# mariohsouto/ProxSDP.jl

Hardware: AMD Instinct MI355X
Metric: PDHG iterations/sec at target rank ~ sqrt(n), Max-Cut SDP n=4000 (tol 1e-4 options) (higher is better)
Workload: dtype f64

## Files before the change

### include/proxsdp_hip.h

```cpp
#ifndef PROXSDP_HIP_H
#define PROXSDP_HIP_H

#include <stdint.h>

#ifdef __cplusplus
extern "C" {
#endif

#define PROXSDP_HIP_ABI_VERSION 10

#define PROXSDP_E_INVALID  (-1)
#define PROXSDP_E_HIP      (-2)
#define PROXSDP_E_NOMEM    (-3)
#define PROXSDP_E_UNSUPP   (-4)
#define PROXSDP_E_INTERNAL (-5)
#define PROXSDP_E_COMM_ABORTED (-6)

#define PROXSDP_STATUS_NOT_CALLED       0
#define PROXSDP_STATUS_OPTIMAL          1
#define PROXSDP_STATUS_TIME_LIMIT       2
#define PROXSDP_STATUS_ITERATION_LIMIT  3
#define PROXSDP_STATUS_INFEAS_OR_UNBND  4
#define PROXSDP_STATUS_DUAL_INFEASIBLE  5
#define PROXSDP_STATUS_INFEASIBLE       6
// ... 265 lines not shown
                            double* packed_out, int32_t* out_rank, double* out_min_eig,
                            int64_t* out_nmatvec, int32_t* out_converged, int32_t* out_fell_back);

int proxsdp_hip_eigsolve(const double* packed, int64_t n, int32_t nev,
                         const proxsdp_options* opt, const double* resid, int32_t cap,
                         double* vals, double* vecs, int32_t* out_count,
                         int32_t* out_converged, int64_t* out_nmatvec, int32_t* out_numiter);

int proxsdp_hip_symv_packed(const double* packed, int64_t n, const double* v, double* y,
                            int32_t repeat, double* ms);

int proxsdp_hip_reconstruct(const double* Z, const double* lambda, int64_t n, int32_t r,
                            double* packed_out, int32_t repeat, double* ms);
int proxsdp_hip_reconstruct_kernel(const double* Z, const double* lambda, int64_t n, int32_t r, int32_t mfma,
                                   double* packed_out, int32_t repeat, double* ms);

int proxsdp_hip_factor_residual(const double* packed, int64_t n, const double* V, int64_t ldv,
                                const double* lam, int32_t r, double* resid2, double* xnorm2);
int proxsdp_hip_factor_residual_kernel(const double* packed, int64_t n, const double* V, int64_t ldv,
                                       const double* lam, int32_t r, double* resid2, double* xnorm2,
                                       int32_t repeat, double* ms);

int proxsdp_hip_full_eig_kernel(const double* packed_in, int64_t n, int32_t sign, double* packed_out,
                                int32_t repeat, double* ms, int32_t* out_rank, int64_t* out_products);

int proxsdp_hip_spmv(const proxsdp_csc* M, int32_t index_base, int32_t transpose,
                     const double* in, double* out);

int proxsdp_hip_primal_update(const double* x, const double* Mty, const double* c, double tau, int64_t n,
                              double* x_out);
// ... 95 lines not shown
```

### proxsdp.jl_amd/binding.py

```python
import ctypes as C
import os
import pathlib
import re

import numpy as np
import scipy.sparse as sp

_HERE = pathlib.Path(__file__).resolve().parent
LIB_PATH = _HERE / "libproxsdp_hip.so"
HEADER_PATH = _HERE.parent / "include" / "proxsdp_hip.h"

TRACE_COLS = 14
TRACE_NAMES = ("iter", "prim_obj", "dual_obj", "gap", "feas", "prim_res", "dual_res",
               "primal_step", "beta", "theta", "target_rank", "trials", "elapsed", "matvecs")


class LibraryNotBuilt(RuntimeError):
    pass


class ProxSDPHipError(RuntimeError):
    def __init__(self, code, msg):
        super().__init__(f"libproxsdp_hip error {code}: {msg}")
        self.code = code
# ... 704 lines not shown
                                   int(p), len(b[0]), float(sigma), _p(out)))
    return out


def reconstruct(Z, lam, n, repeat=0, mfma=-1):
    L = lib()
    Zc = np.asfortranarray(Z, dtype=np.float64)
    lam = _f(lam)
    r = len(lam)
    out = np.zeros(n * (n + 1) // 2)
    ms = f64(0.0)
    _check(L.proxsdp_hip_reconstruct_kernel(Zc.ctypes.data_as(pf64), _p(lam), n, r, mfma, _p(out), repeat, C.byref(ms)))
    return (out, ms.value) if repeat else out


def factor_residual(packed, n, V, lam, repeat=0):
    L = lib()
    x = _f(packed)
    lam = _f(lam)
    r = len(lam)
    Vc = np.asfortranarray(np.asarray(V, dtype=np.float64).reshape(-1, r) if r else np.zeros((n, 0)))
    ldv = Vc.shape[0] if r else n
    if len(x) != n * (n + 1) // 2 or (r and ldv < n):
        raise ValueError("factor_residual: packed / V have the wrong shape")
    r2, x2, ms = f64(0.0), f64(0.0), f64(0.0)
    _check(L.proxsdp_hip_factor_residual_kernel(_p(x), n, Vc.ctypes.data_as(pf64) if r else None, ldv,
                                                _p(lam) if r else None, r, C.byref(r2), C.byref(x2), int(repeat), C.byref(ms)))
    return (r2.value, x2.value, ms.value) if repeat else (r2.value, x2.value)


# ... 238 lines not shown
```

### proxsdp.jl_amd/csrc/capi.hip

```cpp
#include <functional>
#include <memory>
#include <new>
#include <string>

#include "pdhg_loop.hip.hpp"
#include "shard_split.hpp"

namespace {
thread_local std::string g_last_error;

template <typename F>
int guarded(F&& f) {
    try {
        g_last_error.clear();
        return f();
    } catch (const std::bad_alloc&) {
        g_last_error = "out of memory";
        return PROXSDP_E_NOMEM;
    } catch (const proxsdp::HipError& e) {
        g_last_error = e.what();
        return PROXSDP_E_HIP;
    } catch (const std::invalid_argument& e) {
        g_last_error = e.what();
        return PROXSDP_E_INVALID;
// ... 601 lines not shown
            hipEvent_t a, b;
            PX_HIP(hipEventCreate(&a)); PX_HIP(hipEventCreate(&b));
            PX_HIP(hipEventRecord(a, S.stream));
            for (int i = 0; i < repeat; ++i) S.launch_reconstruct(W, Zd.p, (int)n, ld.p, r, x.p);
            PX_HIP(hipEventRecord(b, S.stream));
            PX_HIP(hipEventSynchronize(b));
            float t = 0.f;
            PX_HIP(hipEventElapsedTime(&t, a, b));
            *ms = (double)t / repeat;
            (void)hipEventDestroy(a); (void)hipEventDestroy(b);
        }
        return 0;
    });
}

int proxsdp_hip_factor_residual(const double* packed, int64_t n, const double* V, int64_t ldv,
                                const double* lam, int32_t r, double* resid2, double* xnorm2) {
    return proxsdp_hip_factor_residual_kernel(packed, n, V, ldv, lam, r, resid2, xnorm2, 0, nullptr);
}

int proxsdp_hip_factor_residual_kernel(const double* packed, int64_t n, const double* V, int64_t ldv,
                                       const double* lam, int32_t r, double* resid2, double* xnorm2,
                                       int32_t repeat, double* ms) {
    return guarded([&]() -> int {
        if (!packed || !resid2 || !xnorm2 || (r > 0 && (!V || !lam))) throw std::invalid_argument("NULL buffer");
        if (r < 0) throw std::invalid_argument("r < 0");
        if (n < 1 || n > 46340) throw std::invalid_argument("n out of range");
        if (r > 0 && (ldv < n || ldv >= (int64_t)1 << 31)) throw std::invalid_argument("ldv out of range");
        Engine E(nullptr, n, 2);
        proxsdp::Solver& S = E.S;
// ... 366 lines not shown
```

### proxsdp.jl_amd/csrc/kernels.hip.hpp

```cpp
#pragma once
#include <hip/hip_runtime.h>
#include <cstdint>

namespace proxsdp {
namespace dev {

constexpr int WAVE = 64;
constexpr int TILE = 64;
constexpr int TPB = 256;
constexpr int NWAVE = TPB / WAVE;
constexpr int CPW = TILE / NWAVE;
constexpr double INV_SQRT2 = 0.70710678118654752440;
constexpr double SQRT2 = 1.41421356237309504880;

#ifdef PX_TIMELINE
constexpr int TL_WG = 160, TL_SLOTS = 8, TL_K = 260;
__device__ unsigned long long g_tl[2][TL_K][TL_WG][TL_SLOTS];
#define PX_TL(kind, k, slot)                                                                                   \
    do {                                                                                                       \
        if (threadIdx.x == 0 && (int)blockIdx.x < ::proxsdp::dev::TL_WG && (k) >= 0 && (k) < ::proxsdp::dev::TL_K) { \
            asm volatile("" ::: "memory");                                                                     \
            ::proxsdp::dev::g_tl[kind][k][blockIdx.x][slot] = wall_clock64();                                    \
            asm volatile("" ::: "memory");                                                                     \
        }                                                                                                      \
// ... 1013 lines not shown
                }
            }
        }
    }
    if (FUSE_RES) {
        const double r0 = block_max(m0, s_red);
        const double r1 = block_max(m1, s_red);
        if (threadIdx.x == 0) { respart[blockIdx.x] = r0; respart[rstride + blockIdx.x] = r1; }
    }
}

typedef double v4f64 __attribute__((ext_vector_type(4)));
constexpr int MF_KC = 16;
constexpr int MF_LD = TILE + 16;
template <bool FUSE_RES>
__global__ void __launch_bounds__(TPB)
k_reconstruct_mfma(const double* __restrict__ Z, int ldz, const double* __restrict__ lam, int r,
                   int n, double* __restrict__ xp, const double* __restrict__ xold,
                   const unsigned* __restrict__ mask, long long mask_off, double* __restrict__ respart,
                   int rstride) {
    __shared__ double sA[2][MF_KC][MF_LD];
    __shared__ double sB[2][MF_KC][MF_LD];
    __shared__ double s_red[NWAVE];
    const int nt_ = (n + TILE - 1) / TILE;
    const int tile = xcd_tile(blockIdx.x, nt_ * (nt_ + 1) / 2);
    if (tile >= nt_ * (nt_ + 1) / 2) return;
    int I, J;
    tile_coords(tile, I, J);
    const int lane = threadIdx.x & 63;
    const int w = __builtin_amdgcn_readfirstlane((int)(threadIdx.x >> 6));
    const int l15 = lane & 15, l4 = lane >> 4;
    const int gja = J * TILE + lane, gib = I * TILE + lane;
    const bool ja_ok = gja < n, ib_ok = gib < n;
    const double* __restrict__ zA = Z + (ja_ok ? gja : 0);
    const double* __restrict__ zB = Z + (ib_ok ? gib : 0);
    constexpr int MF_U = MF_KC / NWAVE;
    double pa[MF_U], pb[MF_U];
    auto fetch = [&](int k0) {
#pragma unroll
        for (int u = 0; u < MF_U; ++u) {
            const int k = k0 + w + 4 * u;
            const bool kok = k < r;
            const long long ko = (long long)(kok ? k : 0) * ldz;
            const double lk = lam[kok ? k : 0];
            pa[u] = (kok && ja_ok) ? zA[ko] * lk : 0.0;
            pb[u] = (kok && ib_ok) ? zB[ko] : 0.0;
        }
    };
    auto stash = [&](int buf) {
#pragma unroll
        for (int u = 0; u < MF_U; ++u) { sA[buf][w + 4 * u][lane] = pa[u]; sB[buf][w + 4 * u][lane] = pb[u]; }
    };
    v4f64 acc[4];
#pragma unroll
    for (int b = 0; b < 4; ++b) acc[b] = (v4f64){0.0, 0.0, 0.0, 0.0};
    double xo[16];
    unsigned mk[16];
    if (FUSE_RES) {
#pragma unroll
        for (int reg = 0; reg < 4; ++reg) {
            const int gjc = min(J * TILE + w * 16 + l4 + 4 * reg, n - 1);
#pragma unroll
            for (int b = 0; b < 4; ++b) {
                const int gic = min(I * TILE + b * 16 + l15, gjc);
                const long long idxc = (long long)gjc * (gjc + 1) / 2 + gic;
                xo[reg * 4 + b] = xold[idxc];
                mk[reg * 4 + b] = mask[(mask_off + idxc) >> 5];
            }
        }
    }
    fetch(0);
    stash(0);
    __syncthreads();
    int cur = 0;
    for (int k0 = 0; k0 < r; k0 += MF_KC) {
        const bool more = k0 + MF_KC < r;
        if (more) fetch(k0 + MF_KC);
#pragma unroll
        for (int q = 0; q < MF_KC / 4; ++q) {
            const double a = sA[cur][4 * q + l4][w * 16 + l15];
            double bv[4];
#pragma unroll
            for (int b = 0; b < 4; ++b) bv[b] = sB[cur][4 * q + l4][b * 16 + l15];
#pragma unroll
            for (int b = 0; b < 4; ++b) acc[b] = __builtin_amdgcn_mfma_f64_16x16x4f64(a, bv[b], acc[b], 0, 0, 0);
        }
        if (more) {
            stash(cur ^ 1);
            __syncthreads();
            cur ^= 1;
        }
    }
    double m0 = 0.0, m1 = 0.0;
#pragma unroll
    for (int reg = 0; reg < 4; ++reg) {
        const int gj = J * TILE + w * 16 + l4 + 4 * reg;
#pragma unroll
        for (int b = 0; b < 4; ++b) {
            const int gi = I * TILE + b * 16 + l15;
            if (gj < n && gi <= gj) {
                const long long idx = (long long)gj * (gj + 1) / 2 + gi;
                const double xn = ((gi == gj) ? 1.0 : SQRT2) * acc[b][reg];
                if (FUSE_RES) {
                    const double xov = xo[reg * 4 + b];
                    const long long gidx = mask_off + idx;
                    const bool on = (mk[reg * 4 + b] >> (gidx & 31)) & 1u;
                    if (!on) { m0 = fmax(m0, fabs(xn - xov)); m1 = fmax(m1, fabs(xov)); }
                }
                xp[idx] = xn;
            }
        }
    }
    if (FUSE_RES) {
        const double r0 = block_max(m0, s_red);
        const double r1 = block_max(m1, s_red);
        if (threadIdx.x == 0) { respart[blockIdx.x] = r0; respart[rstride + blockIdx.x] = r1; }
    }
}

__global__ void __launch_bounds__(TPB)
k_factor_residual(const double* __restrict__ xp, int n, const double* __restrict__ V, int ldv,
                  const double* __restrict__ lam, int r, double* __restrict__ part) {
    __shared__ double sA[2][MF_KC][MF_LD];
    __shared__ double sB[2][MF_KC][MF_LD];
    __shared__ double s_red[NWAVE];
    const int nt_ = (n + TILE - 1) / TILE;
    const int tile = xcd_tile(blockIdx.x, nt_ * (nt_ + 1) / 2);
    if (tile >= nt_ * (nt_ + 1) / 2) return;
    int I, J;
    tile_coords(tile, I, J);
// ... 68 lines not shown
                const double d = x - acc[b][reg];
                s0 += wt * (d * d);
                s1 += wt * (x * x);
            }
        }
    }
    const double r0 = block_sum(s0, s_red);
    const double r1 = block_sum(s1, s_red);
    if (threadIdx.x == 0) { part[2 * tile] = r0; part[2 * tile + 1] = r1; }
}

constexpr int RM_LDV = TILE + 16;
constexpr int RM_CG = 16;
__global__ void __launch_bounds__(TPB)
k_lz_rotate_mfma(const double* __restrict__ V, int ldv, int K, const double* __restrict__ U, int ncols,
                 double* __restrict__ out, int ldo, int copy_src, int copy_dst) {
    extern __shared__ double s_mem[];
    const int Kp = (K + 3) & ~3;
    const int ldu = Kp + 2;
    double* s_V = s_mem;
    double* s_U = s_mem + (size_t)Kp * RM_LDV;
    const int lane = threadIdx.x & 63;
    const int w = __builtin_amdgcn_readfirstlane((int)(threadIdx.x >> 6));
    const int l15 = lane & 15, l4 = lane >> 4;
    const int i0 = blockIdx.x * LZ_ROWS;
    const int c0 = blockIdx.y * RM_CG;
    const int cn = min(RM_CG, ncols - c0);
    if (cn > 0) {
        double tu[RM_CG / NWAVE][2];
        for (int jb = 0; jb < Kp; jb += 2 * WAVE) {
#pragma unroll
// ... 26 lines not shown
        }
        __syncthreads();
        v4f64 acc = (v4f64){0.0, 0.0, 0.0, 0.0};
        for (int q = 0; q < Kp / 4; ++q) {
            const double bv = s_V[(4 * q + l4) * RM_LDV + w * 16 + l15];
            const double av = s_U[l15 * ldu + 4 * q + l4];
            acc = __builtin_amdgcn_mfma_f64_16x16x4f64(av, bv, acc, 0, 0, 0);
        }
#pragma unroll
        for (int reg = 0; reg < 4; ++reg) {
            const int c = l4 + 4 * reg;
            if (c < cn) out[(long long)(c0 + c) * ldo + i0 + w * 16 + l15] = acc[reg];
        }
    }
    if (copy_src >= 0 && blockIdx.y == 0 && w == 0) out[(long long)copy_dst * ldo + i0 + lane] = V[(long long)copy_src * ldv + i0 + lane];
}

__global__ void __launch_bounds__(TPB)
k_small_psd_project(double* __restrict__ x, const long long* __restrict__ offs, const int* __restrict__ sides,
                    double tol_psd, int* __restrict__ rank_out, int* __restrict__ npos_out, int nmin, int nmax) {
    extern __shared__ __attribute__((aligned(16))) double sj_mem[];
    __shared__ double s_red[NWAVE];
    __shared__ int s_cnt[2];
    const int n = sides[blockIdx.x];
    if (n < nmin || n > nmax) return;
    double* __restrict__ xp = x + offs[blockIdx.x];
    const int ld = n | 1;
    double* A = sj_mem;
    double* V = A + n * ld;
    double* cs = V + n * ld;
// ... 845 lines not shown
```

### proxsdp.jl_amd/csrc/pdhg_loop.hip.hpp

```cpp
#pragma once
#include "solver.hip.hpp"

namespace proxsdp {

constexpr int PSTRIDE = 2048;
constexpr int NQ = 16;

inline void Solver::spmv(const double* x, double* y) {
    spmv_sparse(x, y);
    if (P.dense()) dense_mv(x, y, true);
}
inline void Solver::spmv_sparse(const double* x, double* y) {
    if (P.Q == 0) return;
    if (csr_wave)
        hipLaunchKernelGGL(dev::k_spmv_csr_wave, dim3(ceil_div(P.Q, dev::NWAVE)), dim3(dev::TPB), 0, stream,
                           csr_ptr.p, csr_col.p, csr_val.p, x, y, (int)P.Q, LONG_ROW);
    else
        hipLaunchKernelGGL(dev::k_spmv_csr_thread, dim3(ceil_div(P.Q, dev::TPB)), dim3(dev::TPB), 0, stream,
                           csr_ptr.p, csr_col.p, csr_val.p, x, y, (int)P.Q, LONG_ROW);
    if (n_seg > 0) {
        hipLaunchKernelGGL(dev::k_spmv_csr_seg, dim3(n_seg), dim3(dev::TPB), 0, stream,
                           seg_lo_d.p, seg_hi_d.p, csr_col.p, csr_val.p, x, segpart_d.p);
        hipLaunchKernelGGL(dev::k_spmv_seg_fin, dim3(ceil_div(n_long, dev::TPB)), dim3(dev::TPB), 0, stream,
                           long_row_d.p, long_ptr_d.p, n_long, segpart_d.p, y);
// ... 142 lines not shown
        return;
    }
    double mn = W.vals[0];
    for (double v : W.vals) mn = std::min(mn, v);
    min_eig[idx] = mn;
    int first = 0, npos = 0;
    if (opt.eigsolver == 1) {
        for (int i = 0; i < nev; ++i) if (W.vals[i] > 0.0) ++npos;
        first = nev - npos;
    } else {
        const int k = std::min(nev, W.converged_eigs);
        for (int i = 0; i < k; ++i) if (W.vals[i] > 0.0) ++npos;
    }
    current_rank[idx] += npos;
    W.last_npos = npos;
    if (npos > 0) W.lam.upload(W.vals.data() + first, npos, stream);
    launch_reconstruct(W, W.Z.p + (size_t)first * W.npad, W.npad, W.lam.p, npos, xo,
                       fuse ? xp : nullptr, fuse ? idx : -1);
    W.recon_r += npos;
    if (W.fop_ok) {
        std::swap(W.Z.p, W.F.p);
        W.F_first = first; W.F_r = npos;
        std::swap(W.lam.p, W.Flam.p);
        std::swap(W.lam.n, W.Flam.n);
        W.have_factors = true; W.x_prev_sparse = false;
    } else {
        W.ritz_first = first; W.ritz_r = npos; W.ritz_ok = true;
    }
    if (W.sign_check_pending) verify_sign_engine(idx, xo);
}

// ... 129 lines not shown
                    if (debug) std::fprintf(stderr, "[proxsdp] certificate failed: block %d iteration %lld theta %.3e scale %.3e npos %d\n",
                                            idx, (long long)iter, theta, cscale, npos);
                    break;
                }
                W.lst.full_eigs_lanczos_certified++;
            }
        }
        int rank = 0;
        for (int i = 0; i < npos; ++i) if (W.vals[i] > opt.tol_psd) ++rank;
        W.use_fop = false;
        if (used_fop) W.lst.fop_projections++;
        W.lst.full_eigs++; W.lst.full_eigs_lanczos++;
        current_rank[idx] = rank;
        min_eig[idx] = 0.0;
        W.last_npos = npos;
        if (npos > 0) W.lam.upload(W.vals.data(), npos, stream);
        launch_reconstruct(W, W.Z.p, W.npad, W.lam.p, npos, xo, fuse ? xp : nullptr, fuse ? idx : -1);
        W.recon_r += npos;
        if (W.fop_ok) {
            std::swap(W.Z.p, W.F.p);
            W.F_first = 0; W.F_r = npos;
            std::swap(W.lam.p, W.Flam.p);
            std::swap(W.lam.n, W.Flam.n);
            W.have_factors = true; W.x_prev_sparse = false;
        } else {
            W.ritz_first = 0; W.ritz_r = npos; W.ritz_ok = true;
        }
        if (verify) {
            if (W.sg_cmp.n < 2) W.sg_cmp.alloc(2);
            W.sg_cmp.zero(stream);
            hipLaunchKernelGGL(dev::k_maxdiff, dim3(grid_for(W.N)), dim3(dev::TPB), 0, stream, (const double*)xo,
// ... 1572 lines not shown
```

### proxsdp.jl_amd/csrc/solver.hip.hpp

```cpp
#pragma once
#include <hip/hip_runtime.h>
#include <hip/hip_ext.h>
#include <array>
#include <memory>
#include <mutex>
#include <condition_variable>
#include <functional>
#include <exception>
#include <rocblas/rocblas.h>
#include <rocsolver/rocsolver.h>

#include <algorithm>
#include <chrono>
#include <cmath>
#include <cstdio>
#include <cstdlib>
#include <cstring>
#include <stdexcept>
#include <string>
#include <thread>
#include <tuple>
#include <type_traits>
#include <utility>
#include <vector>
// ... 108 lines not shown
    }
};

struct EigEvents {
    std::vector<hipEvent_t> e0, e1;
    size_t used = 0;
    std::pair<hipEvent_t, hipEvent_t> acquire() {
        if (used == e0.size()) {
            hipEvent_t a, b;
            PX_HIP(hipEventCreate(&a)); PX_HIP(hipEventCreate(&b));
            e0.push_back(a); e1.push_back(b);
        }
        ++used;
        return {e0[used - 1], e1[used - 1]};
    }
    void harvest(double& ms_sum, int64_t& count) {
        for (size_t s = 0; s < used; ++s) {
            float ms = 0.f;
            if (hipEventElapsedTime(&ms, e0[s], e1[s]) == hipSuccess) { ms_sum += ms; count++; }
        }
        used = 0;
    }
};

struct StreamRef {
    hipStream_t main = nullptr;
    static inline thread_local hipStream_t tl = nullptr;
    operator hipStream_t() const { return tl ? tl : main; }
};

struct LzRun {
    int nev = 0, krylovdim = 0, ld = 0;
    bool arpack = false, positive_part = false;
    double tol = 0.0, step_tol = 0.0;
    long long maxiter = 0;
    std::vector<double> T, Tw, D, U, f, al, be, Qa, da, ea;
// ... 37 lines not shown
    PinnedBuf Ustage[2];
    int ustage_next = 0;
    std::vector<double> vals;
    int count = 0, converged_eigs = 0, numiter = 0, prev_numiter = 1;
    bool converged = false;
    DevBuf<double> F, Flam, tpart, ebuf, apartf;
    DevBuf<int> ell_col, ell_sidx;
    DevBuf<int> wr_ptr, wr_row, wr_lo, wr_hi, ov_col, ov_sidx;
    dev::EllOverflow ov{};
    int ell_w = 0, F_first = 0, F_r = 0;
    bool fop_ok = false;
    bool have_factors = false;
    bool x_prev_sparse = true;
    bool use_fop = false;
    bool ritz_ok = false;
    int ritz_first = 0, ritz_r = 0;
    int last_npos = -1;
    hipStream_t side = nullptr;
    hipEvent_t ev_mid = nullptr, ev_early = nullptr;
    PinnedBuf rec_early;
    SplitEig split;
    int batch_slot = 0;
    bool b1_defer = false;
    int b1_rot_K = 0;
    const double* b1_rot_U = nullptr;
    LzRun lzrun;
    long long fel_served = 0;
    bool fel_disabled = false;
    int fel_cert_fails = 0;
    DevBuf<double> warm_part;
// ... 136 lines not shown
    int block1_lds_cap = 0;
    DevBuf<long long> b1_dbg;
    bool block1_plan(const EigWork& W, int krylovdim, bool split_wanted) const;
    void launch_block1(EigWork& W, const double* xp, int kfirst, int krylovdim, double tol);
    bool sg48_ok = false;
    void launch_symv(EigWork& W, const double* xp, const double* v, bool use_ctl, dev::LanczosCtl* ctl = nullptr);
    void launch_symv_finish(EigWork& W, const double* xp, int kclose, double tol, bool use_carry);
    void launch_reconstruct(EigWork& W, const double* Z, int ldz, const double* lam, int r, double* xp_out,
                            const double* xp_old = nullptr, int blk = -1);
    proxsdp_psd_factors* factors_out = nullptr;
    DevBuf<double> fac_V, fac_lam, fac_part;
    void factor_residual(const double* xp, int n, const double* V, int ldv, const double* lam, int r,
                         double& resid2, double& xnorm2);
    void extract_factors(const std::vector<double>& x);
    void rotate(EigWork& W, int K, const std::vector<double>& U, int ldu, int ncols, double* out, int copy_src, int copy_dst,
                const double* extra, int nextra);

    void test_project(int idx, double* xp, int tr);
    void test_full_eig(const double* xin, double* xout) { current_rank.assign(1, 0); min_eig.assign(1, 0.0); full_eig_project(0, xin, xout, false); }
    long long test_rank() const { return current_rank.empty() ? 0 : current_rank[0]; }
    double test_min_eig() const { return min_eig.empty() ? 0.0 : min_eig[0]; }
    void test_spmv(bool transpose, const double* in, double* out);
    void test_trial_batch(proxsdp_trial_batch& t);
    void test_cone_tail(const double* x, int64_t n, const int64_t* so, const int32_t* sl, int nsoc,
                        const int64_t* oo, int none, double* x_soc, double* gap_in, double* gap_out,
                        double* x_clamp, double* mineig);
    void test_sym_product(proxsdp_sym_product& t);
    void test_sign_unpack(const double* packed, double sentinel, double* A, double* sc);

    bool debug = std::getenv("PROXSDP_HIP_DEBUG") != nullptr;
    proxsdp_options opt;
// ... 475 lines not shown
                                    double& resid2, double& xnorm2) {
    const int nt = ceil_div(n, dev::TILE);
    const int tiles = nt * (nt + 1) / 2;
    if (fac_part.n < (size_t)2 * tiles) fac_part.alloc((size_t)2 * tiles);
    hipLaunchKernelGGL(dev::k_factor_residual, dim3(8 * ceil_div(tiles, 8)), dim3(dev::TPB), 0, stream,
                       xp, n, V, ldv, lam, r, fac_part.p);
    PX_HIP(hipGetLastError());
    std::vector<double> h((size_t)2 * tiles);
    fac_part.download(h.data(), h.size(), stream);
    PX_HIP(hipStreamSynchronize(stream));
    resid2 = 0.0; xnorm2 = 0.0;
    for (int t = 0; t < tiles; ++t) { resid2 += h[2 * t]; xnorm2 += h[2 * t + 1]; }
}

inline void Solver::rotate(EigWork& W, int K, const std::vector<double>& U, int ldu, int ncols,
                           double* out, int copy_src, int copy_dst, const double* extra, int nextra) {
    if (rot_sink != nullptr) {
        RotSink::Req& q = rot_sink->slot[W.batch_slot];
        q.W = &W; q.V = W.V.p; q.out = out; q.K = K; q.ncols = ncols; q.copy_src = copy_src; q.copy_dst = copy_dst;
        q.nextra = std::max(nextra, 0); q.valid = true;
        q.data.resize((size_t)K * std::max(ncols, 0) + (size_t)q.nextra);
        for (int c = 0; c < ncols; ++c)
            for (int j = 0; j < K; ++j) q.data[(size_t)c * K + j] = U[(size_t)c * ldu + j];
        for (int t = 0; t < q.nextra; ++t) q.data[(size_t)K * std::max(ncols, 0) + t] = extra[t];
        return;
    }
    double* tmp = W.Ustage[W.ustage_next].p;
    W.ustage_next ^= 1;
    if ((size_t)K * std::max(ncols, 1) + (size_t)std::max(nextra, 0) > W.ustage_doubles)
        throw std::logic_error("rotation staging buffer too small");
    for (int c = 0; c < ncols; ++c)
        for (int j = 0; j < K; ++j) tmp[(size_t)c * K + j] = U[(size_t)c * ldu + j];
    for (int q = 0; q < nextra; ++q) tmp[(size_t)K * ncols + q] = extra[q];
    if (W.b1_defer && nextra > 0 && K < 32 && copy_src == K && copy_dst == ncols && out == W.Z.p) {
        W.b1_rot_K = K; W.b1_rot_U = tmp;
        W.arrow_p = tmp + (size_t)K * ncols;
        return;
    }
    W.U.upload(tmp, (size_t)K * ncols + (size_t)std::max(nextra, 0), stream);
    if (nextra > 0) W.arrow_p = W.U.p + (size_t)K * ncols;
    if (W.lzrun.wide) {
        if (ncols > 0 || copy_src >= 0)
            hipLaunchKernelGGL(dev::k_lzw_rotate, dim3(W.nt, std::max(1, ceil_div(ncols, dev::LZW_RC))), dim3(dev::TPB), 0, stream,
                               (const double*)W.V.p, W.npad, K, (const double*)W.U.p, ncols, out, W.npad, copy_src, copy_dst);
        return;
    }
    {
        const int Kp = (K + 3) & ~3;
        const size_t lds_m = ((size_t)Kp * dev::RM_LDV + (size_t)dev::RM_CG * (Kp + 2)) * sizeof(double);
        if (K >= 32 && ncols >= 16 && (int)lds_m <= rotate_mfma_lds_cap) {
            hipLaunchKernelGGL(dev::k_lz_rotate_mfma, dim3(W.nt, ceil_div(ncols, dev::RM_CG)), dim3(dev::TPB), lds_m, stream,
                               (const double*)W.V.p, W.npad, K, (const double*)W.U.p, ncols, out, W.npad, copy_src, copy_dst);
            return;
        }
    }
    const int vbytes = K * (dev::LZ_ROWS + 1) * 8;
    const int maxcols = std::max(1, (rotate_lds_cap - vbytes) / (8 * K));
    int c0 = 0;
    do {
        const int cn = std::max(0, std::min(maxcols, ncols - c0));
        const bool last = (c0 + cn >= ncols);
        if (cn > 0 || (last && copy_src >= 0))
            hipLaunchKernelGGL(dev::k_lz_rotate, dim3(W.nt), dim3(dev::TPB), (size_t)K * cn * 8 + vbytes, stream,
                               W.V.p, W.npad, W.n, K, W.U.p + (size_t)c0 * K, K, cn,
                               out + (size_t)c0 * W.npad, W.npad, last ? copy_src : -1, copy_dst - c0);
        c0 += std::max(cn, 1);
    } while (c0 < ncols);
}

// ... 165 lines not shown
    }
    R.kfirst = keep;
    R.presymv = speculated;
    ++R.numiter;
    W.lst.lanczos_restarts++;
}

inline void Solver::lz_finish_run(EigWork& W, LzRun& R) {
    const int K = R.K, nev = R.nev;
    W.numiter = R.numiter;
    if (R.positive_part) {
        if (R.pos_fail || R.pos_count < 0) { W.converged = false; return; }
        W.count = R.pos_count; W.converged_eigs = R.pos_count; W.converged = true;
        W.vals.assign(R.D.begin(), R.D.begin() + R.pos_count);
        if (R.pos_count > 0 && R.merge_active) lz_merge_vectors(W, R, R.pos_count);
        if (R.pos_count > 0) rotate(W, K, R.U, K, R.pos_count, W.Z.p, -1, 0, nullptr, 0);
        return;
    }
    if (R.pos_fail) { W.converged = false; return; }
    if (R.arpack) {
        W.converged_eigs = R.converged;
        if (R.converged < nev) { W.converged = false; return; }
        W.count = nev;
        W.vals.assign(R.D.begin(), R.D.begin() + nev);
        std::reverse(W.vals.begin(), W.vals.end());
        std::vector<double> Ur((size_t)K * nev);
        for (int c = 0; c < nev; ++c)
            for (int r = 0; r < K; ++r) Ur[(size_t)c * K + r] = R.U[(size_t)(nev - 1 - c) * K + r];
        rotate(W, K, Ur, K, nev, W.Z.p, -1, 0, nullptr, 0);
        W.converged = true;
        return;
    }
    int howmany = R.howmany;
    if (R.converged > howmany) howmany = R.converged;
    W.count = howmany;
    W.vals.assign(R.D.begin(), R.D.begin() + howmany);
    W.converged_eigs = R.converged;
    W.converged = (R.converged != 0);
    if (R.merge_active) lz_merge_vectors(W, R, howmany);
    rotate(W, K, R.U, K, howmany, W.Z.p, -1, 0, nullptr, 0);
}

inline void Solver::lanczos_eager(EigWork& W, const double* xp, int nev) {
    LzRun& R = W.lzrun;
    W.use_fop = false;
    if (!lz_init(W, R, nev, false)) return;
    if (R.arpack) throw std::invalid_argument("krylovkit_eager applies to eigsolver = 2 (KrylovKit) only");
    if (R.wide) throw std::invalid_argument("krylovkit_eager: Krylov dimension > 255 is not supported");
    const int kd = R.krylovdim, ld = R.ld;
    const double tol = R.tol;
    lz_launch_begin(W, W.resid.p, W.ctl_p);
    std::vector<double>& T = R.T; std::vector<double>& f = R.f;
    std::vector<double> fstep(2 * dev::MAXK, 0.0);
    int K = 0, kfirst = 0, converged = 0;
    double beta = 0.0;
// ... 144 lines not shown
    std::vector<double> T((size_t)msteps * msteps, 0.0), d(msteps, 0.0);
    for (int j = 0; j < msteps; ++j) {
        if (!(al[j] == al[j]) || !(j + 1 < msteps ? be[j] == be[j] : true)) return false;
        T[(size_t)j * msteps + j] = al[j];
        if (j + 1 < msteps) T[(size_t)j * msteps + j + 1] = T[(size_t)(j + 1) * msteps + j] = be[j];
    }
    if (msteps == 1) d[0] = al[0];
    else if (symeig_dense(msteps, T.data(), d.data(), true) != 0) return false;
    theta_max = d[msteps - 1];
    scale = std::max({std::fabs(d[0]), std::fabs(theta_max), npos > 0 ? std::fabs(W.vals[0]) : 0.0});
    return true;
}

inline void Solver::lanczos(EigWork& W, const double* xp, int nev, bool positive_part) {
    W.ritz_ok = false;
    if (opt.krylovkit_eager && opt.eigsolver != 1 && !positive_part) { lanczos_eager(W, xp, nev); return; }
    LzRun& R = W.lzrun;
    if (!lz_init(W, R, nev, positive_part)) return;
    const int krylovdim = R.krylovdim;
    const double step_tol = R.step_tol;
    const bool wide = R.wide;
    if (wide) W.lst.wide_krylov_projections++;
    if (krylovdim >= 96) QlPool::get().arm();
    dev::LanczosCtl* const ctl = wide ? W.ctlw_p : W.ctl_p;
    const bool warm_start = positive_part ? (opt.lanczos_warm_start >= 0) : (opt.lanczos_warm_start > 0);
    if (!wide && warm_start && W.fop_ok && W.have_factors && W.F_r > 0 && W.tpart.n > 0) {
        const int nb = ceil_div(W.npad, dev::TPB);
        hipLaunchKernelGGL(dev::k_lz_warm_sum, dim3(nb), dim3(dev::TPB), 0, stream,
                           W.V.p, (const double*)(W.F.p + (size_t)W.F_first * W.npad), W.npad, W.F_r,
                           (const double*)W.resid.p, W.npad, W.warm_part.p,
// ... 19 lines not shown
        pool_guard.p = merge_pool.get();
        W.split.M.par = &merge_par;
        W.split.M.nchunk = merge_helpers() + 1;
    }
    if (use_split && W.side == nullptr) {
        PX_HIP(hipStreamCreateWithFlags(&W.side, hipStreamNonBlocking));
        PX_HIP(hipEventCreateWithFlags(&W.ev_mid, hipEventDisableTiming));
        PX_HIP(hipEventCreateWithFlags(&W.ev_early, hipEventDisableTiming));
        W.rec_early.alloc(EigWork::REC_DOUBLES);
    }
    struct DeferGuard {
        EigWork& W;
        DeferGuard(EigWork& w, bool on) : W(w) { W.b1_defer = on; }
        ~DeferGuard() { W.b1_defer = false; }
    };
    while (true) {
        const int kfirst = R.kfirst;
        const int k1 = (kfirst == 0) ? (18 * krylovdim) / 25 : kfirst + 1;
        const bool split_cycle = use_split && k1 >= 1 && k1 <= krylovdim - 2;
        if (wide) {
            for (int k = kfirst; k < krylovdim; ++k) lzw_step(W, xp, k, kfirst, step_tol, R.presymv);
        } else if (blk1) {
            launch_block1(W, xp, kfirst, krylovdim, step_tol);
            R.presymv = false;
        } else {
            for (int k = kfirst; k < krylovdim; ++k) {
                lz_launch_step(W, xp, k, kfirst, step_tol, R.presymv);
                if (split_cycle && k == k1) {
                    PX_HIP(hipEventRecord(W.ev_mid, stream));
                    PX_HIP(hipStreamWaitEvent(W.side, W.ev_mid, 0));
// ... 2 lines not shown
                }
            }
            lz_launch_finish(W, krylovdim - 1, step_tol, krylovdim - 1 > kfirst);
        }
        const bool speculate = !blk1 && (W.prev_numiter > 1 || R.numiter > 1);
        if (speculate) {
            launch_symv(W, xp, W.V.p + (size_t)krylovdim * W.npad, true, ctl);
            count_matvecs(W, -1);
        }
        if (wide) PX_HIP(hipMemcpyAsync(W.recw_pinned.p, W.recw.p, EigWork::RECW_DOUBLES * sizeof(double), hipMemcpyDeviceToHost, stream));
        else PX_HIP(hipMemcpyAsync(W.rec_host, W.rec.p, EigWork::REC_DOUBLES * sizeof(double), hipMemcpyDeviceToHost, stream));
        if (!(split_cycle && lz_split_first(W, R, k1))) lz_prepare_arrow(R);
        const double tdbg0 = debug ? now_s() : 0.0;
        wait_stream();
        if (debug) { dbg_lz[0] += now_s() - tdbg0; dbg_lz[5] += 1.0; }
        if (W.cye_pending) {
            W.cye_pending = false;
            float ms = 0.f;
            if (hipEventElapsedTime(&ms, W.cye[0], W.cye[1]) == hipSuccess) W.lst.cycle_ms += ms;
        }
        W.ev.harvest(W.lst.symv_profiled_ms, W.lst.symv_profiled);
        W.evo.harvest(W.lst.orth_profiled_ms, W.lst.orth_profiled);
        const double tdbg1 = debug ? now_s() : 0.0;
        bool go_on;
        {
            DeferGuard defer(W, blk1);
            go_on = lz_after_cycle(W, R, speculate);
        }
        if (debug) dbg_lz[1] += now_s() - tdbg1;
        if (!go_on) break;
    }
    const double tdbg2 = debug ? now_s() : 0.0;
    lz_finish_run(W, R);
    if (debug) dbg_lz[3] += now_s() - tdbg2;
}

inline void Solver::lzw_step(EigWork& W, const double* xp, int k, int kfirst, double step_tol, bool& presymv) {
    if (k == kfirst && presymv) {
        count_matvecs(W, 1);
    } else {
        launch_symv(W, xp, W.V.p + (size_t)k * W.npad, true, W.ctlw_p);
    }
    presymv = false;
    const dev::LanczosCtl* ctl = W.ctlw_p;
    const int nred = ceil_div(k + 2, dev::TPB);
    hipLaunchKernelGGL(dev::k_lzw_dots, dim3(W.nt), dim3(dev::TPB), 0, stream,
                       (const double*)W.Ppart.p, W.nt, W.npad, (const double*)W.V.p, W.npad, k, W.w.p, W.hpw1.p, ctl);
    hipLaunchKernelGGL(dev::k_lzw_reduce, dim3(nred), dim3(dev::TPB), 0, stream,
                       (const double*)W.hpw1.p, W.pld, W.nt, k, W.hsw1.p, ctl, 0);
// ... 32 lines not shown
    const int nb = (int)blocks.size();
    if (ctx_slot < 0 || ctx_slot >= (int)batch_ctx.size() || !batch_ctx[ctx_slot]) throw std::logic_error("lanczos_batch: no context for this group");
    BatchCtx& C = *batch_ctx[ctx_slot];
    const bool concurrent = StreamRef::tl != nullptr;
    long long steps_local = 0;
    if (nb < 1 || nb > dev::LZB_MAX) throw std::invalid_argument("lanczos_batch: 1..LZB_MAX blocks");
    auto Rq = [&](int q) -> LzRun& { return eig[blocks[q]].lzrun; };
    std::vector<char> live(nb, 0), ran(nb, 0);
    EigWork& W0 = eig[blocks[0]];
    dev::LzBatch B{};
    B.n = W0.n; B.nt = W0.nt; B.npad = W0.npad; B.pld = W0.pld; B.napart = W0.napart; B.nb = nb;
    for (int q = 0; q < nb; ++q) {
        EigWork& W = eig[blocks[q]];
        W.use_fop = false;
        W.ritz_ok = false;
        W.batch_slot = q;
        live[q] = ran[q] = lz_init(W, Rq(q), nevs[q], false) ? 1 : 0;
        if (Rq(q).krylovdim > 63) throw std::invalid_argument("lanczos_batch: krylovdim > 63");
        B.tol = Rq(q).step_tol;
    }
    auto fill = [&](int q) -> dev::LzBlk& {
        EigWork& W = eig[blocks[q]];
        dev::LzBlk& b = B.b[q];
        b.xp = xbase + P.blocks[blocks[q]].off;
        b.Ppart = W.Ppart.p; b.wbuf = W.w.p; b.V = W.V.p; b.hpart1 = W.hpart1.p; b.hpart2 = W.hpart2.p;
        b.hsum = W.hsum1.p; b.alphas = W.alphas_p; b.betas = W.betas_p; b.ctl = W.ctl_p; b.Apart = W.Apart.p;
        b.hred = W.hred.p; b.arrow = W.arrow_p; b.resid = W.resid.p;
        return b;
    };
    const int ntile = 8 * ceil_div(W0.nt * (W0.nt + 1) / 2, 8);
// ... 544 lines not shown
```

Before: 531.8.

## Stage reconstruct results through LDS, piggyback eigenvalue upload on rotate, defer event harvest

Rewrites the MFMA reconstruct epilogue to spill accumulators into shared memory, so each lane writes contiguous packed rows. It also spreads the fused x_old and mask loads across the k-loop, drops the per-element bounds checks in fetch, and raises occupancy through a single reused LDS slab with launch_bounds(TPB,4). Eigenvalues are appended to the rotation coefficient upload and copied by the rotate kernel, which removes a separate host-to-device upload per projection. Event-timing harvests are moved after the host-side Lanczos cycle work so they no longer sit on the critical path. This adds state (lam_delivered) that must stay consistent across code paths, plus a new test entry point.

```diff
diff --git a/include/proxsdp_hip.h b/include/proxsdp_hip.h
--- a/include/proxsdp_hip.h
+++ b/include/proxsdp_hip.h
@@ -303,6 +303,10 @@
                             double* packed_out, int32_t repeat, double* ms);
 int proxsdp_hip_reconstruct_kernel(const double* Z, const double* lambda, int64_t n, int32_t r, int32_t mfma,
                                    double* packed_out, int32_t repeat, double* ms);
+int proxsdp_hip_reconstruct_fused_kernel(const double* Z, int64_t ldz, const double* lambda, int64_t n, int32_t r,
+                                         int32_t mfma, const double* x_old, const uint32_t* mask_words,
+                                         int64_t mask_nwords, int64_t mask_off, double* packed_out, double* m0,
+                                         double* m1, int32_t repeat, double* ms);
 
 int proxsdp_hip_factor_residual(const double* packed, int64_t n, const double* V, int64_t ldv,
                                 const double* lam, int32_t r, double* resid2, double* xnorm2);
diff --git a/proxsdp.jl_amd/binding.py b/proxsdp.jl_amd/binding.py
--- a/proxsdp.jl_amd/binding.py
+++ b/proxsdp.jl_amd/binding.py
@@ -742,6 +742,28 @@
     return (out, ms.value) if repeat else out
 
 
+def reconstruct_fused(Z, lam, n, x_old, mask_words, mask_off=0, repeat=0, mfma=1):
+    L = lib()
+    lam = _f(lam)
+    r = len(lam)
+    Zc = np.asfortranarray(np.asarray(Z, dtype=np.float64).reshape(-1, r) if r else np.zeros((n, 0)))
+    ldz = Zc.shape[0] if r else n
+    xo = _f(x_old)
+    mk = np.ascontiguousarray(mask_words, dtype=np.uint32)
+    N = n * (n + 1) // 2
+    if len(xo) != N or (r and ldz < n):
+        raise ValueError("reconstruct_fused: x_old / Z have the wrong shape")
+    out = np.zeros(N)
+    m0, m1, ms = f64(0.0), f64(0.0), f64(0.0)
+    pu32 = C.POINTER(C.c_uint32)
+    L.proxsdp_hip_reconstruct_fused_kernel.argtypes = [pf64, i64, pf64, i64, i32, i32, pf64, pu32, i64, i64, pf64, pf64,
+                                                       pf64, i32, pf64]
+    _check(L.proxsdp_hip_reconstruct_fused_kernel(Zc.ctypes.data_as(pf64) if r else None, ldz, _p(lam) if r else None,
+                                                  n, r, int(mfma), _p(xo), _p(mk, pu32), len(mk), int(mask_off), _p(out),
+                                                  C.byref(m0), C.byref(m1), int(repeat), C.byref(ms)))
+    return (out, m0.value, m1.value, ms.value) if repeat else (out, m0.value, m1.value)
+
+
 def factor_residual(packed, n, V, lam, repeat=0):
     L = lib()
     x = _f(packed)
diff --git a/proxsdp.jl_amd/csrc/capi.hip b/proxsdp.jl_amd/csrc/capi.hip
--- a/proxsdp.jl_amd/csrc/capi.hip
+++ b/proxsdp.jl_amd/csrc/capi.hip
@@ -639,6 +639,63 @@
     });
 }
 
+int proxsdp_hip_reconstruct_fused_kernel(const double* Z, int64_t ldz, const double* lambda, int64_t n, int32_t r,
+                                         int32_t mfma, const double* x_old, const uint32_t* mask_words,
+                                         int64_t mask_nwords, int64_t mask_off, double* packed_out, double* m0,
+                                         double* m1, int32_t repeat, double* ms) {
+    return guarded([&]() -> int {
+        if ((r > 0 && (!Z || !lambda)) || !x_old || !mask_words || !packed_out || !m0 || !m1)
+            throw std::invalid_argument("NULL buffer");
+        if (r < 0) throw std::invalid_argument("r < 0");
+        if (n < 1 || n > 46340) throw std::invalid_argument("n out of range");
+        if (r > 0 && (ldz < n || ldz >= (int64_t)1 << 31)) throw std::invalid_argument("ldz out of range");
+        const int64_t N = n * (n + 1) / 2;
+        if (mask_off < 0 || mask_nwords < (mask_off + N + 31) / 32) throw std::invalid_argument("mask too short");
+        Engine E(nullptr, n, 2);
+        proxsdp::Solver& S = E.S;
+        const int nt = proxsdp::ceil_div((int)n, proxsdp::dev::TILE);
+        const int grid = 8 * proxsdp::ceil_div(nt * (nt + 1) / 2, 8);
+        const size_t zcount = r > 0 ? (size_t)ldz * (r - 1) + (size_t)n : 0;
+        proxsdp::DevBuf<double> x(N), xo(N), Zd(std::max<size_t>(1, zcount)), ld(std::max(1, r)), part((size_t)2 * grid);
+        proxsdp::DevBuf<unsigned> mk((size_t)mask_nwords);
+        Zd.upload(Z, zcount, S.stream);
+        ld.upload(lambda, r, S.stream);
+        xo.upload(x_old, N, S.stream);
+        mk.upload(mask_words, (size_t)mask_nwords, S.stream);
+        part.zero(S.stream);
+        auto launch = [&]() {
+            if (mfma)
+                hipLaunchKernelGGL(proxsdp::dev::k_reconstruct_mfma<true>, dim3(grid), dim3(proxsdp::dev::TPB), 0, S.stream,
+                                   (const double*)Zd.p, (int)ldz, (const double*)ld.p, (int)r, (int)n, x.p,
+                                   (const double*)xo.p, (const unsigned*)mk.p, (long long)mask_off, part.p, grid);
+            else
+                hipLaunchKernelGGL(proxsdp::dev::k_reconstruct_packed<true>, dim3(grid), dim3(proxsdp::dev::TPB), 0, S.stream,
+                                   (const double*)Zd.p, (int)ldz, (const double*)ld.p, (int)r, (int)n, x.p,
+                                   (const double*)xo.p, (const unsigned*)mk.p, (long long)mask_off, part.p, grid);
+        };
+        launch();
+        std::vector<double> ph((size_t)2 * grid);
+        x.download(packed_out, N, S.stream);
+        part.download(ph.data(), ph.size(), S.stream);
+        PX_HIP(hipStreamSynchronize(S.stream));
+        *m0 = 0.0; *m1 = 0.0;
+        for (int t = 0; t < grid; ++t) { *m0 = std::max(*m0, ph[t]); *m1 = std::max(*m1, ph[grid + t]); }
+        if (repeat > 0 && ms) {
+            hipEvent_t a, b;
+            PX_HIP(hipEventCreate(&a)); PX_HIP(hipEventCreate(&b));
+            PX_HIP(hipEventRecord(a, S.stream));
+            for (int i = 0; i < repeat; ++i) launch();
+            PX_HIP(hipEventRecord(b, S.stream));
+            PX_HIP(hipEventSynchronize(b));
+            float t = 0.f;
+            PX_HIP(hipEventElapsedTime(&t, a, b));
+            *ms = (double)t / repeat;
+            (void)hipEventDestroy(a); (void)hipEventDestroy(b);
+        }
+        return 0;
+    });
+}
+
 int proxsdp_hip_factor_residual(const double* packed, int64_t n, const double* V, int64_t ldv,
                                 const double* lam, int32_t r, double* resid2, double* xnorm2) {
     return proxsdp_hip_factor_residual_kernel(packed, n, V, ldv, lam, r, resid2, xnorm2, 0, nullptr);
diff --git a/proxsdp.jl_amd/csrc/kernels.hip.hpp b/proxsdp.jl_amd/csrc/kernels.hip.hpp
--- a/proxsdp.jl_amd/csrc/kernels.hip.hpp
+++ b/proxsdp.jl_amd/csrc/kernels.hip.hpp
@@ -1051,68 +1051,79 @@
 constexpr int MF_KC = 16;
 constexpr int MF_LD = TILE + 16;
 template <bool FUSE_RES>
-__global__ void __launch_bounds__(TPB)
+__global__ void __launch_bounds__(TPB, 4)
 k_reconstruct_mfma(const double* __restrict__ Z, int ldz, const double* __restrict__ lam, int r,
                    int n, double* __restrict__ xp, const double* __restrict__ xold,
                    const unsigned* __restrict__ mask, long long mask_off, double* __restrict__ respart,
                    int rstride) {
-    __shared__ double sA[2][MF_KC][MF_LD];
-    __shared__ double sB[2][MF_KC][MF_LD];
-    __shared__ double s_red[NWAVE];
+    __shared__ double smem[4 * MF_KC * MF_LD];
+    static_assert(NWAVE * 16 * MF_LD <= 4 * MF_KC * MF_LD && MF_LD >= TILE, "result panels must fit into the slab storage");
+    double (*sA)[MF_KC][MF_LD] = reinterpret_cast<double (*)[MF_KC][MF_LD]>(smem);
+    double (*sB)[MF_KC][MF_LD] = reinterpret_cast<double (*)[MF_KC][MF_LD]>(smem + 2 * MF_KC * MF_LD);
     const int nt_ = (n + TILE - 1) / TILE;
+    const int lane = threadIdx.x & 63;
+    const int w = __builtin_amdgcn_readfirstlane((int)(threadIdx.x >> 6));
+    const int l15 = lane & 15, l4 = lane >> 4;
     const int tile = xcd_tile(blockIdx.x, nt_ * (nt_ + 1) / 2);
     if (tile >= nt_ * (nt_ + 1) / 2) return;
     int I, J;
     tile_coords(tile, I, J);
-    const int lane = threadIdx.x & 63;
-    const int w = __builtin_amdgcn_readfirstlane((int)(threadIdx.x >> 6));
-    const int l15 = lane & 15, l4 = lane >> 4;
     const int gja = J * TILE + lane, gib = I * TILE + lane;
     const bool ja_ok = gja < n, ib_ok = gib < n;
     const double* __restrict__ zA = Z + (ja_ok ? gja : 0);
     const double* __restrict__ zB = Z + (ib_ok ? gib : 0);
     constexpr int MF_U = MF_KC / NWAVE;
-    double pa[MF_U], pb[MF_U];
+    double pa[MF_U], pb[MF_U], pl[MF_U];
+#pragma unroll
+    for (int u = 0; u < MF_U; ++u) pa[u] = pb[u] = pl[u] = 0.0;
     auto fetch = [&](int k0) {
 #pragma unroll
         for (int u = 0; u < MF_U; ++u) {
-            const int k = k0 + w + 4 * u;
-            const bool kok = k < r;
-            const long long ko = (long long)(kok ? k : 0) * ldz;
-            const double lk = lam[kok ? k : 0];
-            pa[u] = (kok && ja_ok) ? zA[ko] * lk : 0.0;
-            pb[u] = (kok && ib_ok) ? zB[ko] : 0.0;
+            const int kc = min(k0 + w + 4 * u, r - 1);
+            const long long ko = (long long)kc * ldz;
+            pl[u] = lam[kc];
+            pa[u] = zA[ko];
+            pb[u] = zB[ko];
         }
     };
-    auto stash = [&](int buf) {
-#pragma unroll
-        for (int u = 0; u < MF_U; ++u) { sA[buf][w + 4 * u][lane] = pa[u]; sB[buf][w + 4 * u][lane] = pb[u]; }
+    auto stash = [&](int buf, int k0) {
+#pragma unroll
+        for (int u = 0; u < MF_U; ++u) {
+            const bool kok = k0 + w + 4 * u < r;
+            const long long ma = (kok && ja_ok) ? -1LL : 0LL, mb = (kok && ib_ok) ? -1LL : 0LL;
+            sA[buf][w + 4 * u][lane] = __longlong_as_double(__double_as_longlong(pa[u] * pl[u]) & ma);
+            sB[buf][w + 4 * u][lane] = __longlong_as_double(__double_as_longlong(pb[u]) & mb);
+        }
     };
     v4f64 acc[4];
 #pragma unroll
     for (int b = 0; b < 4; ++b) acc[b] = (v4f64){0.0, 0.0, 0.0, 0.0};
+    const int gi = I * TILE + lane;
     double xo[16];
     unsigned mk[16];
-    if (FUSE_RES) {
-#pragma unroll
-        for (int reg = 0; reg < 4; ++reg) {
-            const int gjc = min(J * TILE + w * 16 + l4 + 4 * reg, n - 1);
-#pragma unroll
-            for (int b = 0; b < 4; ++b) {
-                const int gic = min(I * TILE + b * 16 + l15, gjc);
-                const long long idxc = (long long)gjc * (gjc + 1) / 2 + gic;
-                xo[reg * 4 + b] = xold[idxc];
-                mk[reg * 4 + b] = mask[(mask_off + idxc) >> 5];
-            }
-        }
-    }
-    fetch(0);
-    stash(0);
+    auto xload = [&](int g) {
+#pragma unroll
+        for (int c = 4 * g; c < 4 * g + 4; ++c) {
+            const int gjc = min(J * TILE + w * 16 + c, n - 1);
+            const long long idxc = (long long)gjc * (gjc + 1) / 2 + min(gi, gjc);
+            xo[c] = xold[idxc];
+            mk[c] = mask[(mask_off + idxc) >> 5];
+        }
+    };
+    int xg = 0;
+    if (r > 0) fetch(0);
+    stash(0, 0);
     __syncthreads();
     int cur = 0;
     for (int k0 = 0; k0 < r; k0 += MF_KC) {
         const bool more = k0 + MF_KC < r;
         if (more) fetch(k0 + MF_KC);
+        if (FUSE_RES) {
+#pragma unroll
+            for (int g = 0; g < 4; ++g)
+                if (xg == g) xload(g);
+            ++xg;
+        }
 #pragma unroll
         for (int q = 0; q < MF_KC / 4; ++q) {
             const double a = sA[cur][4 * q + l4][w * 16 + l15];
@@ -1123,34 +1134,42 @@
             for (int b = 0; b < 4; ++b) acc[b] = __builtin_amdgcn_mfma_f64_16x16x4f64(a, bv[b], acc[b], 0, 0, 0);
         }
         if (more) {
-            stash(cur ^ 1);
+            stash(cur ^ 1, k0 + MF_KC);
             __syncthreads();
             cur ^= 1;
         }
     }
+    if (FUSE_RES) {
+#pragma unroll
+        for (int g = 0; g < 4; ++g)
+            if (xg <= g) xload(g);
+    }
+    __syncthreads();
+    double* __restrict__ T = smem + w * (16 * MF_LD);
+#pragma unroll
+    for (int reg = 0; reg < 4; ++reg)
+#pragma unroll
+        for (int b = 0; b < 4; ++b) T[(l4 + 4 * reg) * MF_LD + b * 16 + l15] = acc[b][reg];
+    __syncthreads();
     double m0 = 0.0, m1 = 0.0;
 #pragma unroll
-    for (int reg = 0; reg < 4; ++reg) {
-        const int gj = J * TILE + w * 16 + l4 + 4 * reg;
-#pragma unroll
-        for (int b = 0; b < 4; ++b) {
-            const int gi = I * TILE + b * 16 + l15;
-            if (gj < n && gi <= gj) {
-                const long long idx = (long long)gj * (gj + 1) / 2 + gi;
-                const double xn = ((gi == gj) ? 1.0 : SQRT2) * acc[b][reg];
-                if (FUSE_RES) {
-                    const double xov = xo[reg * 4 + b];
-                    const long long gidx = mask_off + idx;
-                    const bool on = (mk[reg * 4 + b] >> (gidx & 31)) & 1u;
-                    if (!on) { m0 = fmax(m0, fabs(xn - xov)); m1 = fmax(m1, fabs(xov)); }
-                }
-                xp[idx] = xn;
+    for (int c = 0; c < 16; ++c) {
+        const int gj = J * TILE + w * 16 + c;
+        if (gj < n && gi <= gj) {
+            const long long idx = (long long)gj * (gj + 1) / 2 + gi;
+            const double xn = ((gi == gj) ? 1.0 : SQRT2) * T[c * MF_LD + lane];
+            if (FUSE_RES) {
+                const double xov = xo[c];
+                const long long gidx = mask_off + idx;
+                const bool on = (mk[c] >> (gidx & 31)) & 1u;
+                if (!on) { m0 = fmax(m0, fabs(xn - xov)); m1 = fmax(m1, fabs(xov)); }
             }
+            xp[idx] = xn;
         }
     }
     if (FUSE_RES) {
-        const double r0 = block_max(m0, s_red);
-        const double r1 = block_max(m1, s_red);
+        const double r0 = block_max(m0, smem);
+        const double r1 = block_max(m1, smem);
         if (threadIdx.x == 0) { respart[blockIdx.x] = r0; respart[rstride + blockIdx.x] = r1; }
     }
 }
@@ -1249,7 +1268,8 @@
 constexpr int RM_CG = 16;
 __global__ void __launch_bounds__(TPB)
 k_lz_rotate_mfma(const double* __restrict__ V, int ldv, int K, const double* __restrict__ U, int ncols,
-                 double* __restrict__ out, int ldo, int copy_src, int copy_dst) {
+                 double* __restrict__ out, int ldo, int copy_src, int copy_dst,
+                 const double* __restrict__ lam_src, double* __restrict__ lam_dst, int nlam) {
     extern __shared__ double s_mem[];
     const int Kp = (K + 3) & ~3;
     const int ldu = Kp + 2;
@@ -1306,6 +1326,8 @@
         }
     }
     if (copy_src >= 0 && blockIdx.y == 0 && w == 0) out[(long long)copy_dst * ldo + i0 + lane] = V[(long long)copy_src * ldv + i0 + lane];
+    if (blockIdx.x == 0 && blockIdx.y == 0)
+        for (int t = threadIdx.x; t < nlam; t += TPB) lam_dst[t] = lam_src[t];
 }
 
 __global__ void __launch_bounds__(TPB)
diff --git a/proxsdp.jl_amd/csrc/pdhg_loop.hip.hpp b/proxsdp.jl_amd/csrc/pdhg_loop.hip.hpp
--- a/proxsdp.jl_amd/csrc/pdhg_loop.hip.hpp
+++ b/proxsdp.jl_amd/csrc/pdhg_loop.hip.hpp
@@ -180,7 +180,8 @@
     }
     current_rank[idx] += npos;
     W.last_npos = npos;
-    if (npos > 0) W.lam.upload(W.vals.data() + first, npos, stream);
+    if (npos > 0 && !(W.lam_delivered && first == 0)) W.lam.upload(W.vals.data() + first, npos, stream);
+    W.lam_delivered = false;
     launch_reconstruct(W, W.Z.p + (size_t)first * W.npad, W.npad, W.lam.p, npos, xo,
                        fuse ? xp : nullptr, fuse ? idx : -1);
     W.recon_r += npos;
@@ -340,7 +341,8 @@
         current_rank[idx] = rank;
         min_eig[idx] = 0.0;
         W.last_npos = npos;
-        if (npos > 0) W.lam.upload(W.vals.data(), npos, stream);
+        if (npos > 0 && !W.lam_delivered) W.lam.upload(W.vals.data(), npos, stream);
+        W.lam_delivered = false;
         launch_reconstruct(W, W.Z.p, W.npad, W.lam.p, npos, xo, fuse ? xp : nullptr, fuse ? idx : -1);
         W.recon_r += npos;
         if (W.fop_ok) {
diff --git a/proxsdp.jl_amd/csrc/solver.hip.hpp b/proxsdp.jl_amd/csrc/solver.hip.hpp
--- a/proxsdp.jl_amd/csrc/solver.hip.hpp
+++ b/proxsdp.jl_amd/csrc/solver.hip.hpp
@@ -146,12 +146,15 @@
         ++used;
         return {e0[used - 1], e1[used - 1]};
     }
-    void harvest(double& ms_sum, int64_t& count) {
-        for (size_t s = 0; s < used; ++s) {
+    void harvest(double& ms_sum, int64_t& count) { harvest(ms_sum, count, used); }
+    void harvest(double& ms_sum, int64_t& count, size_t n) {
+        n = std::min(n, used);
+        for (size_t s = 0; s < n; ++s) {
             float ms = 0.f;
             if (hipEventElapsedTime(&ms, e0[s], e1[s]) == hipSuccess) { ms_sum += ms; count++; }
         }
-        used = 0;
+        for (size_t s = n; s < used; ++s) { std::swap(e0[s - n], e0[s]); std::swap(e1[s - n], e1[s]); }
+        used -= n;
     }
 };
 
@@ -219,6 +222,7 @@
     bool x_prev_sparse = true;
     bool use_fop = false;
     bool ritz_ok = false;
+    bool lam_delivered = false;
     int ritz_first = 0, ritz_r = 0;
     int last_npos = -1;
     hipStream_t side = nullptr;
@@ -385,7 +389,7 @@
                          double& resid2, double& xnorm2);
     void extract_factors(const std::vector<double>& x);
     void rotate(EigWork& W, int K, const std::vector<double>& U, int ldu, int ncols, double* out, int copy_src, int copy_dst,
-                const double* extra, int nextra);
+                const double* extra, int nextra, const double* lam = nullptr, int nlam = 0);
 
     void test_project(int idx, double* xp, int tr);
     void test_full_eig(const double* xin, double* xout) { current_rank.assign(1, 0); min_eig.assign(1, 0.0); full_eig_project(0, xin, xout, false); }
@@ -891,7 +895,8 @@
 }
 
 inline void Solver::rotate(EigWork& W, int K, const std::vector<double>& U, int ldu, int ncols,
-                           double* out, int copy_src, int copy_dst, const double* extra, int nextra) {
+                           double* out, int copy_src, int copy_dst, const double* extra, int nextra,
+                           const double* lam, int nlam) {
     if (rot_sink != nullptr) {
         RotSink::Req& q = rot_sink->slot[W.batch_slot];
         q.W = &W; q.V = W.V.p; q.out = out; q.K = K; q.ncols = ncols; q.copy_src = copy_src; q.copy_dst = copy_dst;
@@ -914,7 +919,14 @@
         W.arrow_p = tmp + (size_t)K * ncols;
         return;
     }
-    W.U.upload(tmp, (size_t)K * ncols + (size_t)std::max(nextra, 0), stream);
+    const int Kp = (K + 3) & ~3;
+    const size_t lds_m = ((size_t)Kp * dev::RM_LDV + (size_t)dev::RM_CG * (Kp + 2)) * sizeof(double);
+    const bool mfma_form = !W.lzrun.wide && K >= 32 && ncols >= 16 && (int)lds_m <= rotate_mfma_lds_cap;
+    const size_t nu = (size_t)K * ncols + (size_t)std::max(nextra, 0);
+    const bool deliver = lam != nullptr && nlam > 0 && mfma_form && nextra <= 0 && nu + (size_t)nlam <= W.ustage_doubles &&
+                         (size_t)nlam <= W.lam.n;
+    if (deliver) for (int q = 0; q < nlam; ++q) tmp[nu + q] = lam[q];
+    W.U.upload(tmp, nu + (deliver ? (size_t)nlam : 0), stream);
     if (nextra > 0) W.arrow_p = W.U.p + (size_t)K * ncols;
     if (W.lzrun.wide) {
         if (ncols > 0 || copy_src >= 0)
@@ -922,14 +934,12 @@
                                (const double*)W.V.p, W.npad, K, (const double*)W.U.p, ncols, out, W.npad, copy_src, copy_dst);
         return;
     }
-    {
-        const int Kp = (K + 3) & ~3;
-        const size_t lds_m = ((size_t)Kp * dev::RM_LDV + (size_t)dev::RM_CG * (Kp + 2)) * sizeof(double);
-        if (K >= 32 && ncols >= 16 && (int)lds_m <= rotate_mfma_lds_cap) {
-            hipLaunchKernelGGL(dev::k_lz_rotate_mfma, dim3(W.nt, ceil_div(ncols, dev::RM_CG)), dim3(dev::TPB), lds_m, stream,
-                               (const double*)W.V.p, W.npad, K, (const double*)W.U.p, ncols, out, W.npad, copy_src, copy_dst);
-            return;
-        }
+    if (mfma_form) {
+        hipLaunchKernelGGL(dev::k_lz_rotate_mfma, dim3(W.nt, ceil_div(ncols, dev::RM_CG)), dim3(dev::TPB), lds_m, stream,
+                           (const double*)W.V.p, W.npad, K, (const double*)W.U.p, ncols, out, W.npad, copy_src, copy_dst,
+                           (const double*)(deliver ? W.U.p + nu : nullptr), W.lam.p, deliver ? nlam : 0);
+        W.lam_delivered = deliver;
+        return;
     }
     const int vbytes = K * (dev::LZ_ROWS + 1) * 8;
     const int maxcols = std::max(1, (rotate_lds_cap - vbytes) / (8 * K));
@@ -1125,7 +1135,7 @@
         W.count = R.pos_count; W.converged_eigs = R.pos_count; W.converged = true;
         W.vals.assign(R.D.begin(), R.D.begin() + R.pos_count);
         if (R.pos_count > 0 && R.merge_active) lz_merge_vectors(W, R, R.pos_count);
-        if (R.pos_count > 0) rotate(W, K, R.U, K, R.pos_count, W.Z.p, -1, 0, nullptr, 0);
+        if (R.pos_count > 0) rotate(W, K, R.U, K, R.pos_count, W.Z.p, -1, 0, nullptr, 0, W.vals.data(), R.pos_count);
         return;
     }
     if (R.pos_fail) { W.converged = false; return; }
@@ -1149,7 +1159,7 @@
     W.converged_eigs = R.converged;
     W.converged = (R.converged != 0);
     if (R.merge_active) lz_merge_vectors(W, R, howmany);
-    rotate(W, K, R.U, K, howmany, W.Z.p, -1, 0, nullptr, 0);
+    rotate(W, K, R.U, K, howmany, W.Z.p, -1, 0, nullptr, 0, W.vals.data(), howmany);
 }
 
 inline void Solver::lanczos_eager(EigWork& W, const double* xp, int nev) {
@@ -1324,6 +1334,7 @@
 
 inline void Solver::lanczos(EigWork& W, const double* xp, int nev, bool positive_part) {
     W.ritz_ok = false;
+    W.lam_delivered = false;
     if (opt.krylovkit_eager && opt.eigsolver != 1 && !positive_part) { lanczos_eager(W, xp, nev); return; }
     LzRun& R = W.lzrun;
     if (!lz_init(W, R, nev, positive_part)) return;
@@ -1373,6 +1384,17 @@
         DeferGuard(EigWork& w, bool on) : W(w) { W.b1_defer = on; }
         ~DeferGuard() { W.b1_defer = false; }
     };
+    size_t ev_done = 0, evo_done = 0;
+    bool cye_done = false;
+    auto harvest_done = [&]() {
+        if (cye_done) {
+            float ms = 0.f;
+            if (hipEventElapsedTime(&ms, W.cye[0], W.cye[1]) == hipSuccess) W.lst.cycle_ms += ms;
+        }
+        W.ev.harvest(W.lst.symv_profiled_ms, W.lst.symv_profiled, ev_done);
+        W.evo.harvest(W.lst.orth_profiled_ms, W.lst.orth_profiled, evo_done);
+        ev_done = evo_done = 0; cye_done = false;
+    };
     while (true) {
         const int kfirst = R.kfirst;
         const int k1 = (kfirst == 0) ? (18 * krylovdim) / 25 : kfirst + 1;
@@ -1405,13 +1427,8 @@
         const double tdbg0 = debug ? now_s() : 0.0;
         wait_stream();
         if (debug) { dbg_lz[0] += now_s() - tdbg0; dbg_lz[5] += 1.0; }
-        if (W.cye_pending) {
-            W.cye_pending = false;
-            float ms = 0.f;
-            if (hipEventElapsedTime(&ms, W.cye[0], W.cye[1]) == hipSuccess) W.lst.cycle_ms += ms;
-        }
-        W.ev.harvest(W.lst.symv_profiled_ms, W.lst.symv_profiled);
-        W.evo.harvest(W.lst.orth_profiled_ms, W.lst.orth_profiled);
+        ev_done = W.ev.used; evo_done = W.evo.used;
+        cye_done = W.cye_pending; W.cye_pending = false;
         const double tdbg1 = debug ? now_s() : 0.0;
         bool go_on;
         {
@@ -1420,10 +1437,12 @@
         }
         if (debug) dbg_lz[1] += now_s() - tdbg1;
         if (!go_on) break;
+        harvest_done();
     }
     const double tdbg2 = debug ? now_s() : 0.0;
     lz_finish_run(W, R);
     if (debug) dbg_lz[3] += now_s() - tdbg2;
+    harvest_done();
 }
 
 inline void Solver::lzw_step(EigWork& W, const double* xp, int k, int kfirst, double step_tol, bool& presymv) {
@@ -1486,6 +1505,7 @@
         EigWork& W = eig[blocks[q]];
         W.use_fop = false;
         W.ritz_ok = false;
+        W.lam_delivered = false;
         W.batch_slot = q;
         live[q] = ran[q] = lz_init(W, Rq(q), nevs[q], false) ? 1 : 0;
         if (Rq(q).krylovdim > 63) throw std::invalid_argument("lanczos_batch: krylovdim > 63");
```

New measurement: 538.0, median of 5. Within noise of the previous version (+1.2%).
